# chonlei/neural-ode-ion-channels

Hardware: AMD Instinct MI355X
Metric: trajectories/sec (sinewave protocol, 100k steps) (higher is better)
Workload: dtype f64

## Files before the change

include/ionode.h:

```cpp
#ifndef IONODE_H
#define IONODE_H

#include <stddef.h>
#include <stdint.h>

#ifdef __cplusplus
extern "C" {
#endif

#define IONODE_ABI_VERSION 10

#define IONODE_MODEL_HH2 0
#define IONODE_MODEL_MARKOV6 1
#define IONODE_MODEL_NNF 2
#define IONODE_MODEL_NND 3

#define IONODE_STATUS_OK 0
#define IONODE_STATUS_DT_UNDERFLOW 1
#define IONODE_STATUS_NONFINITE 2
#define IONODE_STATUS_MAX_STEPS 3

#define IONODE_OK 0
#define IONODE_ERR_ARG (-1)
#define IONODE_ERR_UNSUPPORTED (-2)
// ... 22 lines not shown
  double *step_log;
  int64_t step_log_cap;
  double t_eval_t0_hint;
  double t_eval_dt_hint;
  int64_t max_total_steps;
  double *ckpt;
  int32_t ckpt_cap;
  int32_t t_eval_exact;
  const double *sse_ref;
  double *sse_out;
  double max_step;
  const double *v_at_outputs;
  int64_t mlp_image_stride;
  int32_t traj_per_image;
  const int32_t *launch_order;
} ionode_desc;

#define IONODE_DEFAULT_MAX_TOTAL_STEPS 1000000

size_t ionode_mlp_packed_floats(int32_t mlp_layers, int32_t mlp_width);

int ionode_mlp_pack(const float *state_dict_flat, int32_t mlp_layers, int32_t mlp_width, float *packed);

int ionode_dopri5(const ionode_desc *d, const float *mlp_packed, const double *params, const double *prot_v,
                  const double *prot_t, const int32_t *prot_of_traj, const void *y0, const double *t_eval,
                  void *y_out, double *i_out, int32_t *status, int64_t *stats, void *stream);

int ionode_dense_defer_plan(const ionode_desc *d, int32_t want_current, int64_t out[2]);
int ionode_dense_tail_plan(const ionode_desc *d, int32_t want_current, int64_t out[2]);
int ionode_dopri5_deferred(const ionode_desc *d, const float *mlp_packed, const double *params, const double *prot_v,
                           const double *prot_t, const int32_t *prot_of_traj, const void *y0, const double *t_eval,
                           void *y_out, double *i_out, int32_t *status, int64_t *stats, void *stream, void *workspace,
                           int64_t workspace_bytes);

int ionode_protocol_at_outputs(const ionode_desc *d, const double *prot_v, const double *prot_t, const double *t_eval,
                               double *v_out, void *stream);

int ionode_launch_geometry(const ionode_desc *d, int32_t out[4]);

const char *ionode_kernel_name(const ionode_desc *d);

const char *ionode_last_kernel_name(void);

int32_t ionode_lane_wise_from(int32_t model, int32_t mlp_width);

const char *ionode_last_error(void);
int32_t ionode_abi_version(void);


size_t ionode_grad_image_floats(int32_t mlp_layers, int32_t mlp_width);
int ionode_grad_pack(const float *state_dict_flat, int32_t mlp_layers, int32_t mlp_width, float *image);

size_t ionode_grad_record_floats(int32_t mlp_layers, int32_t mlp_width);

int ionode_dopri5_backward(const ionode_desc *d, int32_t it_begin, int32_t it_end, int32_t n_iter, const float *grad_image,
                           const double *params, const double *prot_v, const double *prot_t, const int32_t *prot_of_traj,
                           const double *t_eval, const int32_t *n_accepted, const void *grad_y, double *state,
                           float *records, double *grad_params, double *grad_y0, void *stream);

int ionode_dopri5_backward_sse(const ionode_desc *d, int32_t it_begin, int32_t it_end, int32_t n_iter, const double *params,
                               const double *prot_v, const double *prot_t, const int32_t *prot_of_traj, const double *t_eval,
                               const int32_t *n_accepted, const double *grad_sse, double *state, double *grad_params,
                               double *grad_y0, void *stream);

size_t ionode_grad_packet_doubles(void);
int ionode_dopri5_backward_recompute(const ionode_desc *d, int32_t it_begin, int32_t it_end, int32_t n_iter, const float *grad_image,
// ... 50 lines not shown
```

neural-ode-ion-channels_amd/batched.py:

```python
from dataclasses import dataclass
from typing import Optional

import numpy as np
import torch

from . import capi

_packed_cache = {}
_dev_cache = {}


def _dev(device=None):
    if not torch.cuda.is_available():
        raise capi.IonodeError("no HIP device visible: the integrator has no CPU fallback")
    if device is None:
        return torch.device("cuda", torch.cuda.current_device())
    return torch.device(device)


def _to(x, dtype, dev, key=None):
    if x is None:
        return None
    ck = (key, dtype, str(dev)) if key is not None else None
    if ck is not None and ck in _dev_cache:
# ... 26 lines not shown
        _packed_cache[ck] = img
    return img


@dataclass
class Solution:
    y: torch.Tensor
    i: Optional[torch.Tensor]
    status: torch.Tensor
    stats: Optional[torch.Tensor]
    kernel: str
    sse: Optional[torch.Tensor] = None
    order: Optional[torch.Tensor] = None

    def to_original(self, x):
        if self.order is None:
            return x
        out = torch.empty_like(x)
        out.index_copy_(0, self.order, x)
        return out

    def raise_on_failure(self):
        st = self.status.cpu().numpy()
        bad = np.nonzero(st)[0]
        if bad.size:
            b = int(bad[0])
            raise AssertionError(f"{capi.STATUS_TEXT[int(st[b])]} (trajectory {b}; {bad.size} of {st.size} failed)")


def solve(model, params, prot_v, y0, t_eval, *, weights=None, mlp_layers=0, mlp_width=0, weights_key=None,
          prot_t=None, prot_t0=0.0, prot_dt=1.0, prot_of_traj=None, state_dtype=None, rtol=1e-7, atol=1e-9,
          v_oob=-80.0, max_steps=0, max_total_steps=0, max_step=0.0, current=False, obs_g=1.0, obs_e=-86.0, obs_open_state_only=False,
          tile_waves=0, device=None, step_log=None, t_eval_hint="auto", prot_key=None, t_eval_key=None, sse_ref=None,
          states=True, order=None, traj_per_image=0, launch_order="auto") -> Solution:
    dev = _dev(device)
    t_eval_exact = None
    params_t = _to(params, torch.float64, dev)
    if params_t.dim() == 1:
        params_t = params_t[None, :].contiguous()
    B = params_t.shape[0]
    prot_v_t = _to(prot_v, torch.float64, dev, key=None if prot_key is None else (prot_key, "v"))
    if prot_v_t.dim() == 1:
        prot_v_t = prot_v_t[None, :].contiguous()
    if state_dtype is None:
        state_dtype = y0.dtype if isinstance(y0, torch.Tensor) and y0.dtype in (torch.float32, torch.float64) else torch.float64
    y0_t = _to(y0, state_dtype, dev)
    if y0_t.dim() == 1:
        y0_t = y0_t[None, :]
    if y0_t.shape[0] != B:
        y0_t = y0_t.expand(B, y0_t.shape[1])
    y0_t = y0_t.contiguous()
    pot_t = _to(prot_of_traj, torch.int32, dev)
    order_t = None
    if isinstance(order, str):
        if order != "pilot":
            raise capi.IonodeError("order: a permutation, None or 'pilot'")
        from . import schedule
        te_h = t_eval.detach().cpu().numpy() if isinstance(t_eval, torch.Tensor) else np.asarray(t_eval)
        order = schedule.lpt_order(schedule.pilot_cost(params_t[:, :8], prot_v_t, float(te_h[0]), float(te_h[-1]), prot_t0=prot_t0,
                                                       prot_dt=prot_dt, prot_t=prot_t, prot_of_traj=pot_t, rtol=rtol, atol=atol,
                                                       v_oob=v_oob, device=dev))
    if order is not None:
        order_t = _to(order, torch.int64, dev)
        if order_t.shape != (B,) or int(order_t.min()) < 0 or int(order_t.max()) >= B or \
                not bool(torch.bincount(order_t, minlength=B).eq(1).all()):
            raise capi.IonodeError(f"order must be a permutation of range({B})")
        params_t = params_t.index_select(0, order_t)
# ... 1 lines not shown
        pot_t = (order_t % prot_v_t.shape[0]).to(torch.int32) if pot_t is None else pot_t.index_select(0, order_t)
    if isinstance(t_eval_hint, str) and t_eval_hint == "auto" and not (isinstance(t_eval, torch.Tensor) and t_eval.is_cuda):
        te = t_eval.detach().double().numpy() if isinstance(t_eval, torch.Tensor) else np.asarray(t_eval, dtype=np.float64)
        t_eval_hint = None
        if te.size > 1:
            dth = (te[-1] - te[0]) / (te.size - 1)
            if dth > 0 and np.max(np.abs(te - (te[0] + np.arange(te.size) * dth))) <= 0.5 * dth:
                t_eval_hint = (float(te[0]), float(dth))
                t_eval_exact = bool(np.array_equal(te, te[0] + np.arange(te.size, dtype=np.float64) * dth))
    t_eval_t = _to(t_eval, torch.float64, dev, key=t_eval_key)
    packed = None
    if model in (capi.MODEL_NNF, capi.MODEL_NND):
        if weights is None:
            raise capi.IonodeError("NN models need `weights` (flat fp32 state dict)")
        packed = packed_weights(weights, mlp_layers, mlp_width, dev, key=weights_key)
    if launch_order is not None and not isinstance(launch_order, str):
        if order is not None or traj_per_image:
            raise capi.IonodeError("launch_order cannot be combined with order / traj_per_image")
        lo = _to(launch_order, torch.int64, dev)
        if lo.shape != (B,) or int(lo.min()) < 0 or int(lo.max()) >= B or not bool(torch.bincount(lo, minlength=B).eq(1).all()):
            raise capi.IonodeError(f"launch_order must be a permutation of range({B})")
        launch_order = lo.to(torch.int32).contiguous()
    elif order is not None or traj_per_image:
        launch_order = None
    if traj_per_image and order is not None:
        raise capi.IonodeError("traj_per_image ties trajectories to weight sets by position: it cannot be combined with order")
    r = capi.dopri5(model, params_t, prot_v_t, y0_t, t_eval_t, mlp_packed=packed, traj_per_image=traj_per_image, mlp_layers=mlp_layers,
                    mlp_width=mlp_width, prot_t=_to(prot_t, torch.float64, dev, key=None if prot_key is None else (prot_key, "t")),
                    prot_t0=prot_t0, prot_dt=prot_dt,
                    prot_of_traj=pot_t, rtol=rtol, atol=atol, v_oob=v_oob,
                    max_steps=max_steps, max_total_steps=max_total_steps, max_step=max_step, current=current, obs_g=obs_g, obs_e=obs_e,
                    obs_open_state_only=obs_open_state_only, tile_waves=tile_waves, step_log=step_log,
                    t_eval_hint=t_eval_hint, t_eval_exact=t_eval_exact, sse_ref=_to(sse_ref, torch.float64, dev), states=states,
                    launch_order=launch_order)
    return Solution(y=r["y"], i=r["i"], status=r["status"], stats=r["stats"], kernel=r["kernel"], sse=r["sse"],
                    order=order_t)
```

neural-ode-ion-channels_amd/capi.py:

```python
import ctypes as C
import os
import subprocess

import numpy as np
import torch

_HERE = os.path.dirname(os.path.abspath(__file__))
LIB_PATH = os.environ.get("IONODE_LIB") or os.path.join(_HERE, "libionode.so")

MODEL_HH2, MODEL_MARKOV6, MODEL_NNF, MODEL_NND = 0, 1, 2, 3
STATUS_OK, STATUS_DT_UNDERFLOW, STATUS_NONFINITE, STATUS_MAX_STEPS = 0, 1, 2, 3
STATUS_TEXT = {
    0: "ok",
    1: "underflow in dt",
    2: "non-finite values in state `y`",
    3: "max_num_steps exceeded",
}
ABI_VERSION = 10

EXPORTS = (
    "ionode_abi_version", "ionode_last_error", "ionode_mlp_packed_floats", "ionode_mlp_pack",
    "ionode_launch_geometry", "ionode_kernel_name", "ionode_last_kernel_name", "ionode_lane_wise_from", "ionode_dopri5", "ionode_protocol_at_outputs",
    "ionode_grad_image_floats", "ionode_grad_pack", "ionode_grad_record_floats", "ionode_dopri5_backward", "ionode_dopri5_backward_sse",
    "ionode_grad_packet_doubles", "ionode_dopri5_backward_recompute", "ionode_dopri5_backward_sweep",
    "ionode_dopri5_backward_sse_gc", "ionode_dopri5_backward_recompute_sse", "ionode_dopri5_backward_sweep_sse",
    "ionode_grad_partial_floats", "ionode_grad_reduce", "ionode_grad_reduce_unit", "ionode_grad_reduce_slabs", "ionode_grad_last_error",
    "ionode_regress_step", "ionode_adam_step", "ionode_image_refresh", "ionode_regress_plan",
    "ionode_dense_defer_plan", "ionode_dense_tail_plan", "ionode_dopri5_deferred",
)

SWEEP_BUFFERS = {
    "ionode_dopri5_backward": ("grad_image", "params", "prot_v", "prot_t", "prot_of_traj", "t_eval", "n_accepted", "grad_y", "state",
                               "records", "grad_params", "grad_y0"),
    "ionode_dopri5_backward_sse": ("params", "prot_v", "prot_t", "prot_of_traj", "t_eval", "n_accepted", "grad_sse", "state",
                                   "grad_params", "grad_y0"),
    "ionode_dopri5_backward_recompute": ("grad_image", "params", "prot_v", "prot_t", "prot_of_traj", "t_eval", "n_accepted", "grad_y",
                                         "records", "packets"),
    "ionode_dopri5_backward_sweep": ("grad_image", "params", "prot_v", "prot_t", "prot_of_traj", "t_eval", "n_accepted", "grad_y", "state",
                                     "records", "packets", "grad_params", "grad_y0"),
    "ionode_dopri5_backward_sse_gc": ("prot_v", "prot_t", "prot_of_traj", "t_eval", "n_accepted", "grad_sse", "packets", "sse_grad_y0"),
    "ionode_dopri5_backward_recompute_sse": ("grad_image", "params", "prot_v", "prot_t", "prot_of_traj", "t_eval", "n_accepted", "records",
                                             "packets"),
    "ionode_dopri5_backward_sweep_sse": ("grad_image", "params", "prot_v", "prot_t", "prot_of_traj", "t_eval", "n_accepted", "sse_grad_y0",
                                         "state", "records", "packets", "grad_params", "grad_y0"),
}


def n_state(model):
    return 6 if model == MODEL_MARKOV6 else 2


def n_params(model):
    return 12 if model == MODEL_MARKOV6 else 8


class IonodeDesc(C.Structure):
    _fields_ = [
        ("model", C.c_int32), ("state_f32", C.c_int32), ("n_state", C.c_int32), ("n_out", C.c_int32),
        ("n_traj", C.c_int32), ("n_prot", C.c_int32), ("prot_n", C.c_int32), ("mlp_layers", C.c_int32),
        ("mlp_width", C.c_int32), ("n_params", C.c_int32), ("max_steps", C.c_int64),
        ("prot_t0", C.c_double), ("prot_dt", C.c_double), ("v_oob", C.c_double),
# ... 21 lines not shown
        subprocess.check_call(["make", "-C", csrc, "-s", "clean"])
    subprocess.check_call(["make", "-C", csrc, "-s", f"-j{jobs}"])
    return LIB_PATH


_lib = None


def lib():
    global _lib
    if _lib is None:
        if not os.path.exists(LIB_PATH):
            raise IonodeError(f"{LIB_PATH} is missing: run `python -c 'import __graft_entry__ as g; g.build()'` "
                              "(there is no CPU fallback for the integrator)")
        L = C.CDLL(LIB_PATH)
        L.ionode_abi_version.restype = C.c_int32
        L.ionode_last_error.restype = C.c_char_p
        L.ionode_kernel_name.restype = C.c_char_p
        L.ionode_kernel_name.argtypes = [C.POINTER(IonodeDesc)]
        L.ionode_mlp_packed_floats.restype = C.c_size_t
        L.ionode_mlp_packed_floats.argtypes = [C.c_int32, C.c_int32]
        L.ionode_mlp_pack.restype = C.c_int
        L.ionode_mlp_pack.argtypes = [C.c_void_p, C.c_int32, C.c_int32, C.c_void_p]
        L.ionode_launch_geometry.restype = C.c_int
        L.ionode_launch_geometry.argtypes = [C.POINTER(IonodeDesc), C.POINTER(C.c_int32 * 4)]
        L.ionode_dopri5.restype = C.c_int
        L.ionode_dopri5.argtypes = [C.POINTER(IonodeDesc)] + [C.c_void_p] * 12
        L.ionode_dopri5_deferred.restype = C.c_int
        L.ionode_dopri5_deferred.argtypes = [C.POINTER(IonodeDesc)] + [C.c_void_p] * 13 + [C.c_int64]
        L.ionode_dense_defer_plan.restype = C.c_int
        L.ionode_dense_defer_plan.argtypes = [C.POINTER(IonodeDesc), C.c_int32, C.POINTER(C.c_int64 * 2)]
        L.ionode_dense_tail_plan.restype = C.c_int
        L.ionode_dense_tail_plan.argtypes = [C.POINTER(IonodeDesc), C.c_int32, C.POINTER(C.c_int64 * 2)]
        L.ionode_grad_last_error.restype = C.c_char_p
        for fn in (L.ionode_grad_image_floats, L.ionode_grad_record_floats, L.ionode_grad_partial_floats):
            fn.restype = C.c_size_t
            fn.argtypes = [C.c_int32, C.c_int32]
        L.ionode_grad_pack.restype = C.c_int
        L.ionode_grad_pack.argtypes = [C.c_void_p, C.c_int32, C.c_int32, C.c_void_p]
        L.ionode_grad_packet_doubles.restype = C.c_size_t
        L.ionode_grad_packet_doubles.argtypes = []
        for name, buffers in SWEEP_BUFFERS.items():
            getattr(L, name).restype = C.c_int
            getattr(L, name).argtypes = [C.POINTER(IonodeDesc), C.c_int32, C.c_int32, C.c_int32] + [C.c_void_p] * (len(buffers) + 1)
        L.ionode_grad_reduce.restype = C.c_int
        L.ionode_grad_reduce.argtypes = [C.c_int32, C.c_int32, C.c_void_p, C.c_int64, C.c_int32, C.c_void_p, C.c_void_p]
        L.ionode_grad_reduce_slabs.restype = C.c_int32
        L.ionode_grad_reduce_slabs.argtypes = [C.c_int32, C.c_int32, C.c_int64]
        L.ionode_grad_reduce_unit.restype = C.c_int
        L.ionode_grad_reduce_unit.argtypes = [C.c_int32, C.c_int32, C.c_void_p, C.c_int64, C.c_int32, C.c_void_p, C.c_void_p]
        L.ionode_regress_step.restype = C.c_int
        L.ionode_regress_step.argtypes = [C.c_int32, C.c_int32, C.c_void_p, C.c_void_p, C.c_void_p, C.c_void_p, C.c_int32,
                                          C.c_float, C.c_void_p, C.c_void_p, C.c_int32, C.c_void_p]
        L.ionode_regress_plan.restype = C.c_int
        L.ionode_regress_plan.argtypes = [C.c_int32, C.c_int32, C.POINTER(C.c_int32 * 3)]
        L.ionode_adam_step.restype = C.c_int
        L.ionode_adam_step.argtypes = [C.c_int32, C.c_int32, C.c_int32, C.c_int32, C.c_void_p, C.c_void_p, C.c_void_p,
                                       C.c_void_p, C.c_void_p, C.c_float, C.c_float, C.c_float, C.c_float, C.c_int32,
                                       C.c_void_p, C.c_int32, C.c_void_p]
        L.ionode_image_refresh.restype = C.c_int
        L.ionode_image_refresh.argtypes = [C.c_int32, C.c_int32, C.c_void_p, C.c_void_p, C.c_void_p, C.c_void_p]
        L.ionode_last_kernel_name.restype = C.c_char_p
        L.ionode_last_kernel_name.argtypes = []
        L.ionode_lane_wise_from.restype = C.c_int32
        L.ionode_lane_wise_from.argtypes = [C.c_int32, C.c_int32]
        L.ionode_protocol_at_outputs.restype = C.c_int
# ... 36 lines not shown
        setattr(d, k, v)
    return d


def launch_geometry(desc):
    out = (C.c_int32 * 4)()
    rc = lib().ionode_launch_geometry(C.byref(desc), C.byref(out))
    if rc != 0:
        raise IonodeError(last_error())
    return {"grid": out[0], "block": out[1], "lds_bytes": out[2], "tile_waves": out[3]}


def regress_plan(mlp_layers, mlp_width):
    out = (C.c_int32 * 3)()
    if lib().ionode_regress_plan(int(mlp_layers), int(mlp_width), C.byref(out)) != 0:
        raise IonodeError(lib().ionode_grad_last_error().decode())
    return {"generic": bool(out[0]), "wg_per_cu": out[1], "lds_bytes": out[2]}


def dense_defer_plan(desc, want_current):
    out = (C.c_int64 * 2)()
    if lib().ionode_dense_defer_plan(C.byref(desc), int(bool(want_current)), C.byref(out)) != 0:
        raise IonodeError(last_error())
    return {"capacity": int(out[0]), "workspace_bytes": int(out[1])}


def dense_tail_plan(desc, want_current):
    out = (C.c_int64 * 2)()
    if lib().ionode_dense_tail_plan(C.byref(desc), int(bool(want_current)), C.byref(out)) != 0:
        raise IonodeError(last_error())
    return {"tail_rank": int(out[0]), "usable_capacity": int(out[1])}


def kernel_name(desc):
    return lib().ionode_kernel_name(C.byref(desc)).decode()


def _dev_ptr(t, dtype, name, shape=None):
    if t is None:
        return None
    if not isinstance(t, torch.Tensor) or not t.is_cuda:
        raise IonodeError(f"{name}: expected a CUDA/HIP tensor (the integrator has no CPU path)")
    if t.dtype != dtype or not t.is_contiguous():
        raise IonodeError(f"{name}: expected contiguous {dtype}, got {t.dtype} contiguous={t.is_contiguous()}")
    if shape is not None and tuple(t.shape) != tuple(shape):
        raise IonodeError(f"{name}: expected shape {tuple(shape)}, got {tuple(t.shape)}")
    return C.c_void_p(t.data_ptr())


_order_cache = {}


def _protocol_major(prot_of_traj):
    key = (prot_of_traj.data_ptr(), prot_of_traj._version, int(prot_of_traj.shape[0]), str(prot_of_traj.device))
    hit = _order_cache.get(key)
    if hit is None:
        p = prot_of_traj.to(torch.int64)
        if bool((p[1:] >= p[:-1]).all()):
            hit = (None,)
        else:
            order = torch.argsort(p, stable=True)
            n = int(order.shape[0])
            if n % (64 * 8) == 0:
                order = order.view(8, n // (64 * 8), 64).transpose(0, 1).reshape(-1)
            hit = (order.to(torch.int32).contiguous(),)
        if len(_order_cache) > 8:
            _order_cache.clear()
        _order_cache[key] = hit
    return hit[0]


def dopri5(model, params, prot_v, y0, t_eval, *, mlp_packed=None, mlp_layers=0, mlp_width=0, prot_t=None,
           prot_t0=0.0, prot_dt=1.0, prot_of_traj=None, rtol=1e-7, atol=1e-9, v_oob=-80.0, max_steps=0,
           max_total_steps=0, max_step=0.0, ckpt=None, current=False, obs_g=1.0, obs_e=-86.0, obs_open_state_only=False, tile_waves=0, stats=True,
           step_log=None, t_eval_hint="auto", t_eval_exact=None, sse_ref=None, states=True, out=None, stream=None,
           v_at_outputs="auto", traj_per_image=0, launch_order="auto", workspace=None):
    if not torch.cuda.is_available():
        raise IonodeError("no HIP device visible: ionode has no CPU fallback")
    B, D = y0.shape
    Nt = t_eval.shape[0]
    P, Np = prot_v.shape
    sdt = y0.dtype
    if sdt not in (torch.float32, torch.float64):
        raise IonodeError("y0 must be float32 or float64")
    desc = make_desc(model=model, state_f32=int(sdt == torch.float32), n_state=D, n_out=Nt, n_traj=B, n_prot=P,
                     prot_n=Np, mlp_layers=mlp_layers, mlp_width=mlp_width, n_params=params.shape[1],
                     max_steps=max_steps, max_total_steps=max_total_steps, max_step=max_step, prot_t0=prot_t0, prot_dt=prot_dt, v_oob=v_oob, rtol=rtol, atol=atol,
                     obs_g=obs_g, obs_e=obs_e, obs_open_state_only=int(obs_open_state_only), tile_waves=tile_waves)
    if traj_per_image:
        if mlp_packed is None or mlp_packed.dim() != 2 or mlp_packed.shape[0] * traj_per_image < B or not mlp_packed.is_contiguous():
            raise IonodeError("traj_per_image needs a contiguous mlp_packed [n_images, floats] with n_images * traj_per_image >= B")
        desc.mlp_image_stride, desc.traj_per_image = int(mlp_packed.shape[1]), int(traj_per_image)
    if isinstance(t_eval_hint, str) and t_eval_hint == "auto":
        t_eval_hint = uniform_grid(t_eval)
        if t_eval_hint is not None and t_eval_exact is None:
            t_eval_exact = t_eval_hint[2] == 0.0
    if t_eval_hint is not None and t_eval_hint[1] > 0:
        desc.t_eval_t0_hint, desc.t_eval_dt_hint = float(t_eval_hint[0]), float(t_eval_hint[1])
        if t_eval_exact is None:
            k = torch.arange(Nt, dtype=torch.float64, device=t_eval.device)
            t_eval_exact = bool(torch.equal(t_eval, float(t_eval_hint[0]) + k * float(t_eval_hint[1])))
        desc.t_eval_exact = int(bool(t_eval_exact))
    if isinstance(launch_order, str):
        if launch_order != "auto":
            raise IonodeError("launch_order: None, 'auto' or an int32 device tensor [B]")
        launch_order = None
        lane_from = int(lib().ionode_lane_wise_from(int(model), int(mlp_width or 0)))
        if lane_from > 0 and prot_of_traj is not None and P > 1 and B >= lane_from and not traj_per_image:
            launch_order = _protocol_major(prot_of_traj)
    if launch_order is not None:
        _dev_ptr(launch_order, torch.int32, "launch_order", (B,))
        desc.launch_order = launch_order.data_ptr()
    if ckpt is not None:
        _dev_ptr(ckpt, torch.float64, "ckpt", (B, ckpt.shape[1], ckpt_record_doubles(D)))
        desc.ckpt = ckpt.data_ptr()
        desc.ckpt_cap = ckpt.shape[1]
    if step_log is not None:
        _dev_ptr(step_log, torch.float64, "step_log")
        desc.step_log = step_log.data_ptr()
        desc.step_log_cap = step_log.shape[0]
    dev = y0.device
    if out is None:
        out = {}
    y = out.get("y")
    if y is None and states:
        y = torch.empty((B, Nt, D), dtype=sdt, device=dev)
    sse = None
    if sse_ref is not None:
        _dev_ptr(sse_ref, torch.float64, "sse_ref", (P, Nt))
        sse = out.get("sse")
        if sse is None:
            sse = torch.empty((B,), dtype=torch.float64, device=dev)
        desc.sse_ref, desc.sse_out = sse_ref.data_ptr(), sse.data_ptr()
    elif not states:
        raise IonodeError("states=False needs sse_ref (something must be computed)")
    i_out = out.get("i")
    if current and i_out is None:
        i_out = torch.empty((B, Nt), dtype=torch.float64, device=dev)
    status = out.get("status")
    if status is None:
        status = torch.empty((B,), dtype=torch.int32, device=dev)
    st = out.get("stats")
    if stats and st is None:
        st = torch.empty((B, 4), dtype=torch.int64, device=dev)
    s = stream if stream is not None else torch.cuda.current_stream(dev).cuda_stream
    vtab = None
    if (current or sse_ref is not None) and model in (MODEL_HH2, MODEL_MARKOV6) and v_at_outputs is not None:
        if isinstance(v_at_outputs, str):
            if 4 * P <= B:
                vtab = protocol_at_outputs(desc, prot_v, prot_t, t_eval, stream=s)
        else:
            vtab = v_at_outputs
            _dev_ptr(vtab, torch.float64, "v_at_outputs", (P, Nt))
        if vtab is not None:
            desc.v_at_outputs = vtab.data_ptr()
    ws = None
    if stream is None and prot_t is None and y is not None:
        plan = dense_defer_plan(desc, i_out is not None)
        if plan["capacity"] > 0:
            if workspace is not None:
                _dev_ptr(workspace, torch.uint8, "workspace")
                if workspace.numel() < plan["workspace_bytes"]:
                    raise IonodeError(f"workspace: {workspace.numel()} bytes, the plan asks for {plan['workspace_bytes']}")
            ws = workspace if workspace is not None else torch.empty((plan["workspace_bytes"],), dtype=torch.uint8, device=dev)
    rc = lib().ionode_dopri5_deferred(
        C.byref(desc),
        _dev_ptr(mlp_packed, torch.float32, "mlp_packed"),
        _dev_ptr(params, torch.float64, "params", (B, params.shape[1])),
        _dev_ptr(prot_v, torch.float64, "prot_v"),
        _dev_ptr(prot_t, torch.float64, "prot_t", (Np,)) if prot_t is not None else None,
        _dev_ptr(prot_of_traj, torch.int32, "prot_of_traj", (B,)) if prot_of_traj is not None else None,
        _dev_ptr(y0, sdt, "y0"),
        _dev_ptr(t_eval, torch.float64, "t_eval"),
        _dev_ptr(y, sdt, "y_out", (B, Nt, D)) if y is not None else None,
        _dev_ptr(i_out, torch.float64, "i_out", (B, Nt)) if i_out is not None else None,
        _dev_ptr(status, torch.int32, "status", (B,)),
        _dev_ptr(st, torch.int64, "stats", (B, 4)) if st is not None else None,
        C.c_void_p(s),
        C.c_void_p(ws.data_ptr()) if ws is not None else None,
        ws.numel() if ws is not None else 0,
    )
    if rc != 0:
        raise IonodeError(f"ionode_dopri5 failed ({rc}): {last_error()}")
    return {"y": y, "i": i_out, "status": status, "stats": st, "sse": sse, "desc": desc, "v_at_outputs": vtab,
            "kernel": lib().ionode_last_kernel_name().decode()}


def uniform_grid(t_eval):
    n = int(t_eval.shape[0])
    if n < 2:
        return None
    t0 = t_eval[0]
    dt = (t_eval[n - 1] - t0) / (n - 1)
    dev = (t_eval - (t0 + torch.arange(n, dtype=torch.float64, device=t_eval.device) * dt)).abs().max()
    t0, dt, dev = (float(x) for x in torch.stack([t0, dt, dev]).cpu())
    return (t0, dt, dev) if dt > 0 and dev <= 0.5 * dt else None


def sweep_launch(name, desc, it_begin, it_end, n_iter, stream, **buffers):
    names = SWEEP_BUFFERS[name]
    if set(buffers) != set(names):
        raise TypeError(f"{name}: missing {sorted(set(names) - set(buffers))}, unknown {sorted(set(buffers) - set(names))}")
    ptrs = [None if buffers[n] is None else C.c_void_p(buffers[n].data_ptr()) for n in names]
    rc = getattr(lib(), name)(C.byref(desc), it_begin, it_end, n_iter, *ptrs, C.c_void_p(stream.cuda_stream))
    if rc != 0:
        raise IonodeError(f"{name} failed ({rc}): {lib().ionode_grad_last_error().decode()}")


def protocol_at_outputs(desc, prot_v, prot_t, t_eval, stream=None):
    out = torch.empty((desc.n_prot, desc.n_out), dtype=torch.float64, device=prot_v.device)
    s = stream if stream is not None else torch.cuda.current_stream(prot_v.device).cuda_stream
    rc = lib().ionode_protocol_at_outputs(C.byref(desc), _dev_ptr(prot_v, torch.float64, "prot_v"),
                                          _dev_ptr(prot_t, torch.float64, "prot_t") if prot_t is not None else None,
                                          _dev_ptr(t_eval, torch.float64, "t_eval"), out.data_ptr(), C.c_void_p(s))
    if rc != 0:
        raise IonodeError(f"ionode_protocol_at_outputs failed ({rc}): {last_error()}")
    return out
```

neural-ode-ion-channels_amd/csrc/ionode_capi.hip:

```cpp
#include <algorithm>
#include <cstdio>
#include <cstdlib>
#include <cstring>
#include <vector>

#include "ionode_launch.hpp"

namespace {

constexpr int kTile32From = 8192;
constexpr int kTile4Upto = 1024;
constexpr int kTile1Upto = 256;
constexpr int kTiny64From = 32769;
constexpr int kHh2LaneFrom = 49152;
constexpr int kMarkov6LaneFrom = 24576;

thread_local char g_err[256] = "";
thread_local const char *g_last_kernel = "";

void set_err(const char *fmt, const char *detail = "") { snprintf(g_err, sizeof g_err, fmt, detail); }

inline int np_of(int N) { return 16 * ((N + 15) / 16); }

struct Plan {
  const ionode::Variant *v = nullptr;
  unsigned grid = 0;
  unsigned block = 0;
  size_t lds = 0;
  size_t lw_bytes = 0;
  bool tile_shrink = false;
};


void plan_lane_wise(Plan *pl, size_t tiles, size_t per_wave_bytes) {
  const size_t cap = 160 * 1024, gran = 1280, T = IONODE_LW_TILES_PER_WG;
  pl->lw_bytes = (per_wave_bytes + 15) & ~(size_t)15;
  pl->grid = (unsigned)(8 * ((tiles + 8 * T - 1) / (8 * T)));
  pl->block = (unsigned)(64 * T);
// ... 111 lines not shown
    if (d->traj_per_image % v->traj_per_tile != 0 || d->mlp_image_stride < (int64_t)ionode_mlp_packed_floats(L, d->mlp_width)) {
      set_err("traj_per_image must be a multiple of the tile size (16; 64 with tile_waves = 64; 32 with tile_waves = 8) and mlp_image_stride at least one packed image");
      return IONODE_ERR_ARG;
    }
  }
  return IONODE_OK;
}

struct DeferPlan {
  int64_t cap = 0, bytes = 0;
};
DeferPlan plan_defer(const ionode_desc *d, const Plan &pl, bool want_i) {
  DeferPlan p;
  if (!pl.v->defer || d->sse_out != nullptr || d->n_state != 2) return p;
  const char *sw = getenv("IONODE_DEFER_DENSE");
  if (sw != nullptr && sw[0] != '\0' && atoi(sw) == 0) return p;
  using Rec = ionode::DenseRecord<2>;
  const int64_t B = d->n_traj, Nt = d->n_out;
  const char *fc = getenv("IONODE_DEFER_DENSE_CAP");
  int64_t cap = (fc != nullptr && fc[0] != '\0') ? atoll(fc) : 0;
  const bool forced = cap > 0;
  if (!forced) {
    const int64_t out_bytes = B * Nt * 2 * (d->state_f32 ? 4 : 8) + (want_i ? B * Nt * 8 : 0);
    cap = (out_bytes / 4) / (B * Rec::BYTES);
  }
  cap = std::min<int64_t>(cap, Nt - 1);
  if (cap < (forced ? 1 : 64)) return p;
  p.cap = cap;
  p.bytes = (int64_t)Rec::workspace_bytes(B, cap);
  return p;
}

constexpr int64_t kDeferTailEighths = 5;
struct TailPlan {
  int64_t rank = 0, fill = 0;
};
TailPlan plan_tail(const Plan &pl, const DeferPlan &dp) {
  TailPlan t;
  t.fill = dp.cap;
  if (dp.cap < 2) return t;
  const int64_t tiles = (int64_t)pl.grid;
  t.rank = tiles * kDeferTailEighths / 8;
  const char *fr = getenv("IONODE_DEFER_TAIL_RANK");
  if (fr != nullptr && fr[0] != '\0') t.rank = std::max<int64_t>(0, std::min<int64_t>(atoll(fr), tiles));
  const char *sw = getenv("IONODE_DEFER_TAIL");
  if (sw != nullptr && sw[0] != '\0') {
    if (strcmp(sw, "all") == 0) t.rank = tiles;
    else if (atoi(sw) == 0) t.rank = 0;
  }
  if (t.rank > 0) t.fill = dp.cap - 1;
  return t;
}

int make_plan(const ionode_desc *d, Plan *pl, bool want_current = false, bool explicit_grid = false) {
  if (!d) { set_err("null descriptor"); return IONODE_ERR_ARG; }
#ifdef IONODE_STAMPS
  const bool has_step_log = false;
#else
  const bool has_step_log = d->step_log != nullptr;
#endif
  const bool mlp = d->model == IONODE_MODEL_NNF || d->model == IONODE_MODEL_NND;
  const int D = d->model == IONODE_MODEL_MARKOV6 ? 6 : 2;
  if (d->model < 0 || d->model > 3) { set_err("unknown model"); return IONODE_ERR_ARG; }
  if (d->n_state != D) { set_err("n_state does not match model"); return IONODE_ERR_ARG; }
  if (d->n_traj < 1 || d->n_out < 1 || d->n_prot < 1 || d->prot_n < 2) { set_err("empty batch / grid / protocol"); return IONODE_ERR_ARG; }
  if (d->n_params < (D == 6 ? 12 : 8)) { set_err("n_params too small for model"); return IONODE_ERR_ARG; }
  if (!(d->rtol > 0) || !(d->atol >= 0) || !(d->prot_dt > 0)) { set_err("rtol/atol/prot_dt must be positive"); return IONODE_ERR_ARG; }
  const Ask k = {want_current, explicit_grid, has_step_log};
  return mlp ? plan_mlp(d, pl, k) : plan_closed(d, pl, k, D);
}

}

namespace ionode {
__global__ void __launch_bounds__(256) ionode_protocol_at_outputs_kernel(const KArgs a, double *__restrict__ v_out) {
  const long long n = (long long)a.P * a.Nt;
  for (long long e = (long long)blockIdx.x * 256 + threadIdx.x; e < n; e += (long long)gridDim.x * 256) {
    const int p = (int)(e / a.Nt), k = (int)(e - (long long)p * a.Nt);
    double v;
    protocol_v(a, a.prot_v + (size_t)p * a.Np, a.t_eval[k], v);
    v_out[e] = v;
  }
}
}
// ... 225 lines not shown
  return IONODE_OK;
}

const char *ionode_kernel_name(const ionode_desc *d) {
  Plan pl;
  if (make_plan(d, &pl, d && (d->sse_out != nullptr || d->v_at_outputs != nullptr)) != IONODE_OK) return "";
  return pl.v->name;
}

const char *ionode_last_kernel_name(void) { return g_last_kernel; }

int32_t ionode_lane_wise_from(int32_t model, int32_t mlp_width) { return lane_wise_from(model, mlp_width); }

int ionode_dense_defer_plan(const ionode_desc *d, int32_t want_current, int64_t out[2]) {
  Plan pl;
  const int rc = make_plan(d, &pl, want_current != 0 || (d && d->sse_out != nullptr));
  if (rc != IONODE_OK) return rc;
  const DeferPlan dp = plan_defer(d, pl, want_current != 0);
  out[0] = dp.cap;
  out[1] = dp.bytes;
  return IONODE_OK;
}

int ionode_dense_tail_plan(const ionode_desc *d, int32_t want_current, int64_t out[2]) {
  Plan pl;
  const int rc = make_plan(d, &pl, want_current != 0 || (d && d->sse_out != nullptr));
  if (rc != IONODE_OK) return rc;
  const TailPlan tp = plan_tail(pl, plan_defer(d, pl, want_current != 0));
  out[0] = tp.rank;
  out[1] = tp.fill;
  return IONODE_OK;
}

}

namespace {

int dopri5_impl(const ionode_desc *d, const float *mlp_packed, const double *params, const double *prot_v,
                const double *prot_t, const int32_t *prot_of_traj, const void *y0, const double *t_eval,
                void *y_out, double *i_out, int32_t *status, int64_t *stats, void *stream, void *workspace, int64_t workspace_bytes) {
  Plan pl;
  const int rc = make_plan(d, &pl, i_out != nullptr || d->sse_out != nullptr, prot_t != nullptr);
  if (rc != IONODE_OK) return rc;
  const bool mlp = d->model == IONODE_MODEL_NNF || d->model == IONODE_MODEL_NND;
  if (!params || !prot_v || !y0 || !t_eval || (!y_out && !d->sse_out) || !status || (mlp && !mlp_packed)) {
    set_err("ionode_dopri5: required buffer is NULL");
    return IONODE_ERR_ARG;
  }
  if (d->sse_out && (!d->sse_ref || !(d->t_eval_dt_hint > 0.0) || d->n_out < 2)) {
    set_err("fused objective: sse_out needs sse_ref and the output-grid hint (t_eval_dt_hint > 0)");
    return IONODE_ERR_ARG;
  }
  ionode::KArgs a;
  memset(&a, 0, sizeof a);
  a.mlp = mlp_packed; a.params = params; a.prot_v = prot_v; a.prot_t = prot_t; a.prot_of_traj = prot_of_traj;
  a.y0 = y0; a.t_eval = t_eval; a.y_out = y_out; a.i_out = i_out; a.status = status; a.stats = stats;
  a.B = d->n_traj; a.Nt = d->n_out; a.P = d->n_prot; a.Np = d->prot_n; a.n_params = d->n_params;
  if (mlp) { a.L = d->mlp_layers; a.N = d->mlp_width; a.NP = np_of(d->mlp_width); a.NT = a.NP / 16; }
  a.max_steps = d->max_steps > 0 ? d->max_steps : (int64_t)2147483647;
  a.max_total = d->max_total_steps > 0 ? d->max_total_steps
                                       : (d->max_total_steps == 0 ? (int64_t)IONODE_DEFAULT_MAX_TOTAL_STEPS : INT64_MAX);
  a.ckpt = d->ckpt; a.ckpt_cap = d->ckpt ? d->ckpt_cap : 0;
  if (d->ckpt && d->ckpt_cap < 1) { set_err("ckpt given with ckpt_cap < 1"); return IONODE_ERR_ARG; }
  a.prot_rdt = 1.0 / d->prot_dt;
  a.dt_max = d->max_step > 0.0 ? d->max_step : __builtin_inf();
  a.prot_t0 = d->prot_t0; a.prot_dt = d->prot_dt; a.v_oob = d->v_oob; a.rtol = d->rtol; a.atol = d->atol;
  a.obs_g = d->obs_g; a.obs_e = d->obs_e; a.obs_open = d->obs_open_state_only;
  a.step_log = d->step_log; a.step_log_cap = d->step_log ? d->step_log_cap : 0;
  a.sse_ref = d->sse_ref; a.sse_out = d->sse_out; a.v_tab = d->v_at_outputs;
  if (mlp && d->traj_per_image > 0) { a.mlp_stride = d->mlp_image_stride; a.traj_per_img = d->traj_per_image; }
  if (d->launch_order) {
    if (a.traj_per_img > 0) { set_err("launch_order cannot be combined with traj_per_image (tiles of an image must stay together)"); return IONODE_ERR_ARG; }
    a.order = d->launch_order;
  }
  a.lw_bytes = (int32_t)pl.lw_bytes;
  a.te_t0 = d->t_eval_t0_hint; a.te_dt = (d->t_eval_dt_hint > 0.0 && d->n_out > 1) ? d->t_eval_dt_hint : 0.0;
  a.te_rdt = a.te_dt > 0.0 ? 1.0 / a.te_dt : 0.0;
  a.te_exact = (a.te_dt > 0.0 && d->t_eval_exact) ? 1 : 0;
  a.tile_shrink = pl.tile_shrink ? 1 : 0;
  DeferPlan dp;
  if (workspace != nullptr && prot_t == nullptr && y_out != nullptr) dp = plan_defer(d, pl, i_out != nullptr);
  if (dp.cap > 0) {
    if (workspace_bytes < dp.bytes || (reinterpret_cast<uintptr_t>(workspace) & 15) != 0) {
      set_err("ionode_dopri5_deferred: workspace smaller than ionode_dense_defer_plan() asks for, or not 16-byte aligned");
      return IONODE_ERR_ARG;
    }
    a.defer_count = static_cast<int32_t *>(workspace);
    a.defer_rec = reinterpret_cast<double *>(static_cast<unsigned char *>(workspace) + ionode::DenseRecord<2>::records_offset(d->n_traj));
    a.defer_cap = (int32_t)dp.cap;
    const TailPlan tp = plan_tail(pl, dp);
    a.defer_fill = (int32_t)tp.fill;
    a.defer_tail_rank = (int32_t)tp.rank;
    if (tp.rank > 0) {
      a.defer_tail = reinterpret_cast<int32_t *>(a.defer_rec + ((size_t)d->n_traj * (size_t)dp.cap - 1) * ionode::DenseRecord<2>::ROW);
      const hipError_t em = hipMemsetAsync(a.defer_tail, 0, ionode::DenseRecord<2>::BYTES, reinterpret_cast<hipStream_t>(stream));
      if (em != hipSuccess) { set_err("hipMemsetAsync failed: %s", hipGetErrorString(em)); return IONODE_ERR_LAUNCH; }
    }
  }
  hipError_t e = pl.v->fn(a, pl.grid, pl.lds, reinterpret_cast<hipStream_t>(stream));
  if (e != hipSuccess) { set_err("kernel launch failed: %s", hipGetErrorString(e)); return IONODE_ERR_LAUNCH; }
  if (dp.cap > 0) {
    const int64_t blocks = std::min<int64_t>((dp.cap + ionode::kExpandRecordsPerWg - 1) / ionode::kExpandRecordsPerWg, ionode::kExpandMaxBlocks);
    const dim3 grid((unsigned)std::min<int64_t>((int64_t)d->n_traj * blocks, ionode::kExpandGrid));
    if (d->state_f32) hipLaunchKernelGGL((ionode::ionode_dense_expand_kernel<float, 2>), grid, dim3(256), 0, reinterpret_cast<hipStream_t>(stream), a);
    else hipLaunchKernelGGL((ionode::ionode_dense_expand_kernel<double, 2>), grid, dim3(256), 0, reinterpret_cast<hipStream_t>(stream), a);
    e = hipGetLastError();
    if (e != hipSuccess) { set_err("kernel launch failed: %s", hipGetErrorString(e)); return IONODE_ERR_LAUNCH; }
  }
  g_last_kernel = pl.v->name;
  return IONODE_OK;
}

}

extern "C" {

int ionode_dopri5(const ionode_desc *d, const float *mlp_packed, const double *params, const double *prot_v,
                  const double *prot_t, const int32_t *prot_of_traj, const void *y0, const double *t_eval,
                  void *y_out, double *i_out, int32_t *status, int64_t *stats, void *stream) {
  return dopri5_impl(d, mlp_packed, params, prot_v, prot_t, prot_of_traj, y0, t_eval, y_out, i_out, status, stats, stream, nullptr, 0);
}

int ionode_dopri5_deferred(const ionode_desc *d, const float *mlp_packed, const double *params, const double *prot_v,
                           const double *prot_t, const int32_t *prot_of_traj, const void *y0, const double *t_eval,
                           void *y_out, double *i_out, int32_t *status, int64_t *stats, void *stream, void *workspace,
                           int64_t workspace_bytes) {
  return dopri5_impl(d, mlp_packed, params, prot_v, prot_t, prot_of_traj, y0, t_eval, y_out, i_out, status, stats, stream, workspace,
                     workspace_bytes);
}

int ionode_protocol_at_outputs(const ionode_desc *d, const double *prot_v, const double *prot_t, const double *t_eval,
                               double *v_out, void *stream) {
  if (!d || !prot_v || !t_eval || !v_out) { set_err("ionode_protocol_at_outputs: required buffer is NULL"); return IONODE_ERR_ARG; }
  if (d->n_out < 1 || d->n_prot < 1 || d->prot_n < 2 || !(d->prot_dt > 0)) { set_err("ionode_protocol_at_outputs: empty grid / protocol"); return IONODE_ERR_ARG; }
  ionode::KArgs a;
  memset(&a, 0, sizeof a);
  a.prot_v = prot_v; a.prot_t = prot_t; a.t_eval = t_eval; a.Nt = d->n_out; a.P = d->n_prot; a.Np = d->prot_n;
  a.prot_t0 = d->prot_t0; a.prot_dt = d->prot_dt; a.prot_rdt = 1.0 / d->prot_dt; a.v_oob = d->v_oob;
  const long long n = (long long)a.P * a.Nt;
  const unsigned grid = (unsigned)((n + 255) / 256 > 65536 ? 65536 : (n + 255) / 256);
  hipLaunchKernelGGL(ionode::ionode_protocol_at_outputs_kernel, dim3(grid), dim3(256), 0, reinterpret_cast<hipStream_t>(stream), a, v_out);
  const hipError_t e = hipGetLastError();
  if (e != hipSuccess) { set_err("kernel launch failed: %s", hipGetErrorString(e)); return IONODE_ERR_LAUNCH; }
  return IONODE_OK;
}

}
```

Measured before the change: 12700.

## Compose launch order from pilot solve or step-count cost for tile load balance

Adds a cost-based launch ordering path. When no explicit order is given, the Python entry either reuses step counts from caller stats or runs a low-tolerance pilot HH2 solve to estimate per-trajectory cost. A one-workgroup bitonic sort kernel then places the heaviest trajectories into the first slots of each 16-wide tile and fills the rest with light ones, which balances work across tiles and shrinking lanes. This adds an extra pilot integration and a sort launch per call, and the pilot only uses the HH2 model as its cost proxy.

```diff
diff --git a/include/ionode.h b/include/ionode.h
--- a/include/ionode.h
+++ b/include/ionode.h
@@ -78,6 +78,15 @@
                            const double *prot_t, const int32_t *prot_of_traj, const void *y0, const double *t_eval,
                            void *y_out, double *i_out, int32_t *status, int64_t *stats, void *stream, void *workspace,
                            int64_t workspace_bytes);
+
+int ionode_dopri5_composed(const ionode_desc *d, const float *mlp_packed, const double *params, const double *prot_v,
+                           const double *prot_t, const int32_t *prot_of_traj, const void *y0, const double *t_eval,
+                           void *y_out, double *i_out, int32_t *status, int64_t *stats, void *stream, void *workspace,
+                           int64_t workspace_bytes, int32_t cost_source);
+int ionode_compose_tail_plan(const ionode_desc *d, int32_t want_current, int32_t cost_source, int64_t out[2]);
+int ionode_compose_plan(const ionode_desc *d, int32_t want_current, int32_t out[2]);
+int ionode_compose_order(const void *cost, int32_t cost_is_int64, int64_t cost_stride, int32_t n_traj, int32_t *order, void *stream);
+int ionode_compose_order_host(const double *cost, int32_t n_traj, int32_t *order);
 
 int ionode_protocol_at_outputs(const ionode_desc *d, const double *prot_v, const double *prot_t, const double *t_eval,
                                double *v_out, void *stream);
diff --git a/neural-ode-ion-channels_amd/batched.py b/neural-ode-ion-channels_amd/batched.py
--- a/neural-ode-ion-channels_amd/batched.py
+++ b/neural-ode-ion-channels_amd/batched.py
@@ -82,7 +82,7 @@
           prot_t=None, prot_t0=0.0, prot_dt=1.0, prot_of_traj=None, state_dtype=None, rtol=1e-7, atol=1e-9,
           v_oob=-80.0, max_steps=0, max_total_steps=0, max_step=0.0, current=False, obs_g=1.0, obs_e=-86.0, obs_open_state_only=False,
           tile_waves=0, device=None, step_log=None, t_eval_hint="auto", prot_key=None, t_eval_key=None, sse_ref=None,
-          states=True, order=None, traj_per_image=0, launch_order="auto") -> Solution:
+          states=True, order=None, traj_per_image=0, launch_order="auto", cost_hint="auto") -> Solution:
     dev = _dev(device)
     t_eval_exact = None
     params_t = _to(params, torch.float64, dev)
@@ -150,6 +150,6 @@
                     max_steps=max_steps, max_total_steps=max_total_steps, max_step=max_step, current=current, obs_g=obs_g, obs_e=obs_e,
                     obs_open_state_only=obs_open_state_only, tile_waves=tile_waves, step_log=step_log,
                     t_eval_hint=t_eval_hint, t_eval_exact=t_eval_exact, sse_ref=_to(sse_ref, torch.float64, dev), states=states,
-                    launch_order=launch_order)
+                    launch_order=launch_order, cost_hint=cost_hint)
     return Solution(y=r["y"], i=r["i"], status=r["status"], stats=r["stats"], kernel=r["kernel"], sse=r["sse"],
                     order=order_t)
diff --git a/neural-ode-ion-channels_amd/capi.py b/neural-ode-ion-channels_amd/capi.py
--- a/neural-ode-ion-channels_amd/capi.py
+++ b/neural-ode-ion-channels_amd/capi.py
@@ -27,6 +27,7 @@
     "ionode_grad_partial_floats", "ionode_grad_reduce", "ionode_grad_reduce_unit", "ionode_grad_reduce_slabs", "ionode_grad_last_error",
     "ionode_regress_step", "ionode_adam_step", "ionode_image_refresh", "ionode_regress_plan",
     "ionode_dense_defer_plan", "ionode_dense_tail_plan", "ionode_dopri5_deferred",
+    "ionode_compose_plan", "ionode_compose_order", "ionode_compose_order_host", "ionode_dopri5_composed", "ionode_compose_tail_plan",
 )
 
 SWEEP_BUFFERS = {
@@ -114,6 +115,16 @@
         L.ionode_dense_defer_plan.argtypes = [C.POINTER(IonodeDesc), C.c_int32, C.POINTER(C.c_int64 * 2)]
         L.ionode_dense_tail_plan.restype = C.c_int
         L.ionode_dense_tail_plan.argtypes = [C.POINTER(IonodeDesc), C.c_int32, C.POINTER(C.c_int64 * 2)]
+        L.ionode_compose_plan.restype = C.c_int
+        L.ionode_compose_plan.argtypes = [C.POINTER(IonodeDesc), C.c_int32, C.POINTER(C.c_int32 * 2)]
+        L.ionode_compose_order.restype = C.c_int
+        L.ionode_compose_order.argtypes = [C.c_void_p, C.c_int32, C.c_int64, C.c_int32, C.c_void_p, C.c_void_p]
+        L.ionode_dopri5_composed.restype = C.c_int
+        L.ionode_dopri5_composed.argtypes = [C.POINTER(IonodeDesc)] + [C.c_void_p] * 13 + [C.c_int64, C.c_int32]
+        L.ionode_compose_tail_plan.restype = C.c_int
+        L.ionode_compose_tail_plan.argtypes = [C.POINTER(IonodeDesc), C.c_int32, C.c_int32, C.POINTER(C.c_int64 * 2)]
+        L.ionode_compose_order_host.restype = C.c_int
+        L.ionode_compose_order_host.argtypes = [C.c_void_p, C.c_int32, C.c_void_p]
         L.ionode_grad_last_error.restype = C.c_char_p
         for fn in (L.ionode_grad_image_floats, L.ionode_grad_record_floats, L.ionode_grad_partial_floats):
             fn.restype = C.c_size_t
@@ -216,6 +227,48 @@
     return {"tail_rank": int(out[0]), "usable_capacity": int(out[1])}
 
 
+COST_SOURCE = {None: 0, "pilot": 1, "hint": 2, "explicit": 2}
+COMPOSE_SOURCES = {0: "off", 1: "pilot", 2: "hint", 3: "auto"}
+PILOT_RTOL, PILOT_ATOL = 1e-4, 1e-6
+PILOT_MAX_ATTEMPTS = 100000
+
+
+def compose_plan(desc, want_current):
+    out = (C.c_int32 * 2)()
+    if lib().ionode_compose_plan(C.byref(desc), int(bool(want_current)), C.byref(out)) != 0:
+        raise IonodeError(last_error())
+    return {"compose": bool(out[0]), "source": COMPOSE_SOURCES[int(out[1])]}
+
+
+def compose_tail_plan(desc, want_current, composed):
+    out = (C.c_int64 * 2)()
+    if lib().ionode_compose_tail_plan(C.byref(desc), int(bool(want_current)), COST_SOURCE[composed], C.byref(out)) != 0:
+        raise IonodeError(last_error())
+    return {"tail_rank": int(out[0]), "usable_capacity": int(out[1])}
+
+
+def compose_order_host(cost):
+    c = np.ascontiguousarray(np.asarray(cost, dtype=np.float64).reshape(-1))
+    order = np.empty(c.size, dtype=np.int32)
+    if lib().ionode_compose_order_host(c.ctypes.data, int(c.size), order.ctypes.data) != 0:
+        raise IonodeError(last_error())
+    return order
+
+
+def compose_order(cost, stream=None):
+    if not isinstance(cost, torch.Tensor) or not cost.is_cuda or cost.dim() != 1 or cost.dtype not in (torch.float64, torch.int64) \
+            or cost.shape[0] < 1 or (cost.shape[0] > 1 and cost.stride(0) < 1):
+        raise IonodeError("cost: expected a 1-D float64 or int64 CUDA/HIP tensor with a positive stride")
+    B = int(cost.shape[0])
+    order = torch.empty((B,), dtype=torch.int32, device=cost.device)
+    s = stream if stream is not None else torch.cuda.current_stream(cost.device).cuda_stream
+    rc = lib().ionode_compose_order(C.c_void_p(cost.data_ptr()), int(cost.dtype == torch.int64), max(1, int(cost.stride(0))), B,
+                                    C.c_void_p(order.data_ptr()), C.c_void_p(s))
+    if rc != 0:
+        raise IonodeError(f"ionode_compose_order failed ({rc}): {last_error()}")
+    return order
+
+
 def kernel_name(desc):
     return lib().ionode_kernel_name(C.byref(desc)).decode()
 
@@ -258,7 +311,7 @@
            prot_t0=0.0, prot_dt=1.0, prot_of_traj=None, rtol=1e-7, atol=1e-9, v_oob=-80.0, max_steps=0,
            max_total_steps=0, max_step=0.0, ckpt=None, current=False, obs_g=1.0, obs_e=-86.0, obs_open_state_only=False, tile_waves=0, stats=True,
            step_log=None, t_eval_hint="auto", t_eval_exact=None, sse_ref=None, states=True, out=None, stream=None,
-           v_at_outputs="auto", traj_per_image=0, launch_order="auto", workspace=None):
+           v_at_outputs="auto", traj_per_image=0, launch_order="auto", workspace=None, cost_hint="auto"):
     if not torch.cuda.is_available():
         raise IonodeError("no HIP device visible: ionode has no CPU fallback")
     B, D = y0.shape
@@ -285,7 +338,8 @@
             k = torch.arange(Nt, dtype=torch.float64, device=t_eval.device)
             t_eval_exact = bool(torch.equal(t_eval, float(t_eval_hint[0]) + k * float(t_eval_hint[1])))
         desc.t_eval_exact = int(bool(t_eval_exact))
-    if isinstance(launch_order, str):
+    auto_order = isinstance(launch_order, str)
+    if auto_order:
         if launch_order != "auto":
             raise IonodeError("launch_order: None, 'auto' or an int32 device tensor [B]")
         launch_order = None
@@ -325,6 +379,7 @@
     if status is None:
         status = torch.empty((B,), dtype=torch.int32, device=dev)
     st = out.get("stats")
+    stats_from_caller = st is not None
     if stats and st is None:
         st = torch.empty((B, 4), dtype=torch.int64, device=dev)
     s = stream if stream is not None else torch.cuda.current_stream(dev).cuda_stream
@@ -338,6 +393,28 @@
             _dev_ptr(vtab, torch.float64, "v_at_outputs", (P, Nt))
         if vtab is not None:
             desc.v_at_outputs = vtab.data_ptr()
+    composed = None
+    if auto_order and launch_order is None and cost_hint is not None and stream is None and prot_t is None and Nt >= 2:
+        cp = compose_plan(desc, i_out is not None)
+        if cp["compose"]:
+            want = cost_hint if not (isinstance(cost_hint, str) and cost_hint == "auto" and tile_waves) else None
+            cost = None
+            if isinstance(want, torch.Tensor):
+                if tuple(want.shape) != (B,):
+                    raise IonodeError(f"cost_hint: expected shape {(B,)}, got {tuple(want.shape)}")
+                cost, composed = want, "explicit"
+            elif want is not None and want not in ("auto", "pilot", "hint"):
+                raise IonodeError("cost_hint: None, 'auto', 'pilot', 'hint' or a device tensor [B]")
+            elif want in ("auto", "hint") and cp["source"] in ("hint", "auto") and stats_from_caller and _dev_ptr(st, torch.int64, "stats", (B, 4)):
+                cost, composed = st[:, 2], "hint"
+            elif want in ("auto", "pilot") and cp["source"] in ("pilot", "auto"):
+                pilot = dopri5(MODEL_HH2, params, prot_v, y0, torch.stack((t_eval[0], t_eval[Nt - 1])), prot_t0=prot_t0, prot_dt=prot_dt,
+                               prot_of_traj=prot_of_traj, rtol=PILOT_RTOL, atol=PILOT_ATOL, v_oob=v_oob, t_eval_hint=None,
+                               max_total_steps=PILOT_MAX_ATTEMPTS, launch_order=None, cost_hint=None)
+                cost, composed = pilot["stats"][:, 2], "pilot"
+            if cost is not None:
+                launch_order = compose_order(cost)
+                desc.launch_order = launch_order.data_ptr()
     ws = None
     if stream is None and prot_t is None and y is not None:
         plan = dense_defer_plan(desc, i_out is not None)
@@ -347,7 +424,7 @@
                 if workspace.numel() < plan["workspace_bytes"]:
                     raise IonodeError(f"workspace: {workspace.numel()} bytes, the plan asks for {plan['workspace_bytes']}")
             ws = workspace if workspace is not None else torch.empty((plan["workspace_bytes"],), dtype=torch.uint8, device=dev)
-    rc = lib().ionode_dopri5_deferred(
+    rc = lib().ionode_dopri5_composed(
         C.byref(desc),
         _dev_ptr(mlp_packed, torch.float32, "mlp_packed"),
         _dev_ptr(params, torch.float64, "params", (B, params.shape[1])),
@@ -363,11 +440,12 @@
         C.c_void_p(s),
         C.c_void_p(ws.data_ptr()) if ws is not None else None,
         ws.numel() if ws is not None else 0,
+        COST_SOURCE[composed],
     )
     if rc != 0:
         raise IonodeError(f"ionode_dopri5 failed ({rc}): {last_error()}")
     return {"y": y, "i": i_out, "status": status, "stats": st, "sse": sse, "desc": desc, "v_at_outputs": vtab,
-            "kernel": lib().ionode_last_kernel_name().decode()}
+            "launch_order": launch_order, "composed": composed, "kernel": lib().ionode_last_kernel_name().decode()}
 
 
 def uniform_grid(t_eval):
diff --git a/neural-ode-ion-channels_amd/csrc/ionode_capi.hip b/neural-ode-ion-channels_amd/csrc/ionode_capi.hip
--- a/neural-ode-ion-channels_amd/csrc/ionode_capi.hip
+++ b/neural-ode-ion-channels_amd/csrc/ionode_capi.hip
@@ -4,6 +4,7 @@
 #include <cstring>
 #include <vector>
 
+#include "ionode_compose.hpp"
 #include "ionode_launch.hpp"
 
 namespace {
@@ -181,15 +182,17 @@
 }
 
 constexpr int64_t kDeferTailEighths = 5;
+constexpr int64_t kDeferTailEighthsPilot = 5;
+constexpr int64_t kDeferTailEighthsCounts = 5;
 struct TailPlan {
   int64_t rank = 0, fill = 0;
 };
-TailPlan plan_tail(const Plan &pl, const DeferPlan &dp) {
+TailPlan plan_tail(const Plan &pl, const DeferPlan &dp, int cost_source = 0) {
   TailPlan t;
   t.fill = dp.cap;
   if (dp.cap < 2) return t;
   const int64_t tiles = (int64_t)pl.grid;
-  t.rank = tiles * kDeferTailEighths / 8;
+  t.rank = tiles * (cost_source == 1 ? kDeferTailEighthsPilot : cost_source == 2 ? kDeferTailEighthsCounts : kDeferTailEighths) / 8;
   const char *fr = getenv("IONODE_DEFER_TAIL_RANK");
   if (fr != nullptr && fr[0] != '\0') t.rank = std::max<int64_t>(0, std::min<int64_t>(atoll(fr), tiles));
   const char *sw = getenv("IONODE_DEFER_TAIL");
@@ -199,6 +202,27 @@
   }
   if (t.rank > 0) t.fill = dp.cap - 1;
   return t;
+}
+
+enum ComposeSource : int32_t { kComposeOff = 0, kComposePilot = 1, kComposeHint = 2, kComposeAuto = 3 };
+ComposeSource compose_source() {
+  const char *sw = getenv("IONODE_COMPOSE");
+  if (sw == nullptr || sw[0] == '\0') return kComposeAuto;
+  if (strcmp(sw, "pilot") == 0) return kComposePilot;
+  if (strcmp(sw, "hint") == 0) return kComposeHint;
+  return atoi(sw) == 0 ? kComposeOff : kComposeAuto;
+}
+int compute_units_now() {
+  int dev = 0, n = 0;
+  if (hipGetDevice(&dev) != hipSuccess || hipDeviceGetAttribute(&n, hipDeviceAttributeMultiprocessorCount, dev) != hipSuccess || n < 1) {
+    (void)hipGetLastError();
+    return 256;
+  }
+  return n;
+}
+bool plan_compose(const ionode_desc *d, const Plan &pl) {
+  return pl.v->shrink && pl.tile_shrink && pl.v->traj_per_tile == ionode::kComposeTile && d->traj_per_image <= 0 &&
+         d->launch_order == nullptr && d->n_traj <= ionode::kComposeMaxB && (int64_t)pl.grid <= (int64_t)compute_units_now();
 }
 
 int make_plan(const ionode_desc *d, Plan *pl, bool want_current = false, bool explicit_grid = false) {
@@ -490,13 +514,63 @@
   return IONODE_OK;
 }
 
+
+int ionode_compose_tail_plan(const ionode_desc *d, int32_t want_current, int32_t cost_source, int64_t out[2]) {
+  Plan pl;
+  const int rc = make_plan(d, &pl, want_current != 0 || (d && d->sse_out != nullptr));
+  if (rc != IONODE_OK) return rc;
+  if (cost_source < 0 || cost_source > 2) { set_err("cost_source: 0 (not composed), 1 (pilot) or 2 (counts)"); return IONODE_ERR_ARG; }
+  const TailPlan tp = plan_tail(pl, plan_defer(d, pl, want_current != 0), d->launch_order ? cost_source : 0);
+  out[0] = tp.rank;
+  out[1] = tp.fill;
+  return IONODE_OK;
+}
+
+int ionode_compose_plan(const ionode_desc *d, int32_t want_current, int32_t out[2]) {
+  Plan pl;
+  const int rc = make_plan(d, &pl, want_current != 0 || (d && d->sse_out != nullptr));
+  if (rc != IONODE_OK) return rc;
+  const ComposeSource src = compose_source();
+  out[0] = (src != kComposeOff && plan_compose(d, pl)) ? 1 : 0;
+  out[1] = (int32_t)src;
+  return IONODE_OK;
+}
+
+int ionode_compose_order_host(const double *cost, int32_t n_traj, int32_t *order) {
+  if (!cost || !order || n_traj < 1) { set_err("ionode_compose_order_host: bad argument"); return IONODE_ERR_ARG; }
+  std::vector<int32_t> idx((size_t)n_traj);
+  std::vector<double> c((size_t)n_traj);
+  for (int32_t i = 0; i < n_traj; ++i) { idx[i] = i; c[i] = ionode::compose_cost(cost[i]); }
+  std::sort(idx.begin(), idx.end(), [&](int32_t x, int32_t y) { return ionode::compose_before(c[x], x, c[y], y); });
+  const bool flat = c[idx[0]] == c[idx[n_traj - 1]];
+  for (int32_t p = 0; p < n_traj; ++p) order[flat ? p : ionode::compose_slot(p, n_traj)] = idx[p];
+  return IONODE_OK;
+}
+
+int ionode_compose_order(const void *cost, int32_t cost_is_int64, int64_t cost_stride, int32_t n_traj, int32_t *order, void *stream) {
+  if (!cost || !order || n_traj < 1 || cost_stride < 1) { set_err("ionode_compose_order: bad argument"); return IONODE_ERR_ARG; }
+  if (n_traj > ionode::kComposeMaxB) { set_err("ionode_compose_order: more trajectories than the one-workgroup sort holds (8192)"); return IONODE_ERR_UNSUPPORTED; }
+  const size_t lds = ionode::compose_lds_bytes(n_traj);
+  auto kern = cost_is_int64 ? ionode::ionode_compose_kernel<1> : ionode::ionode_compose_kernel<0>;
+  if (lds > 64 * 1024) {
+    const hipError_t ea = hipFuncSetAttribute(reinterpret_cast<const void *>(kern), hipFuncAttributeMaxDynamicSharedMemorySize, (int)lds);
+    if (ea != hipSuccess) { set_err("kernel launch failed: %s", hipGetErrorString(ea)); return IONODE_ERR_LAUNCH; }
+  }
+  hipLaunchKernelGGL(kern, dim3(1), dim3(ionode::kComposeThreads), lds, reinterpret_cast<hipStream_t>(stream), cost, (long long)cost_stride,
+                     (int)n_traj, order);
+  const hipError_t e = hipGetLastError();
+  if (e != hipSuccess) { set_err("kernel launch failed: %s", hipGetErrorString(e)); return IONODE_ERR_LAUNCH; }
+  return IONODE_OK;
+}
+
 }
 
 namespace {
 
 int dopri5_impl(const ionode_desc *d, const float *mlp_packed, const double *params, const double *prot_v,
                 const double *prot_t, const int32_t *prot_of_traj, const void *y0, const double *t_eval,
-                void *y_out, double *i_out, int32_t *status, int64_t *stats, void *stream, void *workspace, int64_t workspace_bytes) {
+                void *y_out, double *i_out, int32_t *status, int64_t *stats, void *stream, void *workspace, int64_t workspace_bytes,
+                int cost_source = 0) {
   Plan pl;
   const int rc = make_plan(d, &pl, i_out != nullptr || d->sse_out != nullptr, prot_t != nullptr);
   if (rc != IONODE_OK) return rc;
@@ -546,7 +620,7 @@
     a.defer_count = static_cast<int32_t *>(workspace);
     a.defer_rec = reinterpret_cast<double *>(static_cast<unsigned char *>(workspace) + ionode::DenseRecord<2>::records_offset(d->n_traj));
     a.defer_cap = (int32_t)dp.cap;
-    const TailPlan tp = plan_tail(pl, dp);
+    const TailPlan tp = plan_tail(pl, dp, d->launch_order ? cost_source : 0);
     a.defer_fill = (int32_t)tp.fill;
     a.defer_tail_rank = (int32_t)tp.rank;
     if (tp.rank > 0) {
@@ -585,6 +659,15 @@
                            int64_t workspace_bytes) {
   return dopri5_impl(d, mlp_packed, params, prot_v, prot_t, prot_of_traj, y0, t_eval, y_out, i_out, status, stats, stream, workspace,
                      workspace_bytes);
+}
+
+int ionode_dopri5_composed(const ionode_desc *d, const float *mlp_packed, const double *params, const double *prot_v,
+                           const double *prot_t, const int32_t *prot_of_traj, const void *y0, const double *t_eval,
+                           void *y_out, double *i_out, int32_t *status, int64_t *stats, void *stream, void *workspace,
+                           int64_t workspace_bytes, int32_t cost_source) {
+  if (cost_source < 0 || cost_source > 2) { set_err("cost_source: 0 (not composed), 1 (pilot) or 2 (counts)"); return IONODE_ERR_ARG; }
+  return dopri5_impl(d, mlp_packed, params, prot_v, prot_t, prot_of_traj, y0, t_eval, y_out, i_out, status, stats, stream, workspace,
+                     workspace_bytes, cost_source);
 }
 
 int ionode_protocol_at_outputs(const ionode_desc *d, const double *prot_v, const double *prot_t, const double *t_eval,
diff --git a/neural-ode-ion-channels_amd/csrc/ionode_compose.hpp b/neural-ode-ion-channels_amd/csrc/ionode_compose.hpp
--- /dev/null
+++ b/neural-ode-ion-channels_amd/csrc/ionode_compose.hpp
@@ -0,0 +1,72 @@
+#pragma once
+
+#include <hip/hip_runtime.h>
+#include <stdint.h>
+
+namespace ionode {
+
+constexpr int kComposeTile = 16;
+constexpr int kComposeHeavy = 4;
+constexpr int kComposeMaxB = 8192;
+constexpr int kComposeThreads = 1024;
+
+__host__ __device__ inline double compose_cost(double c) { return (c >= 0.0 && c <= 1.7976931348623157e308) ? c : 0.0; }
+
+__host__ __device__ inline bool compose_before(double ca, int ia, double cb, int ib) { return ca > cb || (ca == cb && ia < ib); }
+
+__host__ __device__ inline int compose_slot(int p, int B) {
+  const int NT = (B + kComposeTile - 1) / kComposeTile;
+  const int r = B - kComposeTile * (NT - 1);
+  const int nH = kComposeHeavy * (NT - 1) + (r < kComposeHeavy ? r : kComposeHeavy);
+  const int LPT = kComposeTile - kComposeHeavy;
+  if (p < nH) return kComposeTile * (p / kComposeHeavy) + p % kComposeHeavy;
+  const int q = B - 1 - p;
+  if (q < LPT * (NT - 1)) return kComposeTile * (q / LPT) + kComposeHeavy + q % LPT;
+  return kComposeTile * (NT - 1) + kComposeHeavy + (q - LPT * (NT - 1));
+}
+
+__host__ __device__ inline int compose_padded(int B) {
+  int n = 1;
+  while (n < B) n <<= 1;
+  return n;
+}
+inline size_t compose_lds_bytes(int B) { return (size_t)compose_padded(B) * (sizeof(double) + sizeof(int32_t)); }
+
+template <int I64>
+__global__ void __launch_bounds__(kComposeThreads) ionode_compose_kernel(const void *__restrict__ cost, long long stride, int B,
+                                                                         int32_t *__restrict__ order) {
+  extern __shared__ __attribute__((aligned(16))) unsigned char compose_smem[];
+  const int n = compose_padded(B);
+  double *const key = reinterpret_cast<double *>(compose_smem);
+  int32_t *const idx = reinterpret_cast<int32_t *>(key + n);
+  for (int i = threadIdx.x; i < n; i += kComposeThreads) {
+    double c = -1.0;
+    if (i < B) {
+      if constexpr (I64) c = compose_cost((double)static_cast<const long long *>(cost)[(long long)i * stride]);
+      else c = compose_cost(static_cast<const double *>(cost)[(long long)i * stride]);
+    }
+    key[i] = c;
+    idx[i] = i;
+  }
+  __syncthreads();
+  for (int k = 2; k <= n; k <<= 1)
+    for (int j = k >> 1; j > 0; j >>= 1) {
+      for (int i = threadIdx.x; i < n; i += kComposeThreads) {
+        const int l = i ^ j;
+        if (l > i) {
+          const double ci = key[i], cl = key[l];
+          const int ii = idx[i], il = idx[l];
+          const bool first = (i & k) == 0;
+          if (first ? compose_before(cl, il, ci, ii) : compose_before(ci, ii, cl, il)) {
+            key[i] = cl; key[l] = ci;
+            idx[i] = il; idx[l] = ii;
+          }
+        }
+      }
+      __syncthreads();
+    }
+  const bool flat = key[0] == key[B - 1];
+  for (int p = threadIdx.x; p < B; p += kComposeThreads) order[flat ? p : compose_slot(p, B)] = idx[p];
+}
+
+}
```

Measured after the change: 13630, median of 6. +7.4%, better.
